# KrishnaswamyLab/MELD

Measured on AMD Instinct MI355X. Metric: cells/sec through MELD.fit_transform (kNN+Chebyshev), higher is better.
Workload: dtype f64

## Files before the change

include/meld_hip.h:

```cpp
#ifndef MELD_HIP_H
#define MELD_HIP_H

#include <stddef.h>
#include <stdint.h>

#ifdef __cplusplus
extern "C" {
#endif

#define MELD_OK 0
#define MELD_ERR_INVALID (-1)
#define MELD_ERR_UNSUPPORTED (-2)
#define MELD_ERR_HIP (-3)

typedef void* meld_stream_t;

int meld_abi_version(void);
const char* meld_last_error(void);
int meld_device_count(void);


int meld_knn_padded_dim(int d);
int meld_knn_tile_refs(void);
int meld_knn_block_queries(void);
// ... 82 lines not shown
                                 const void* Rt16, const float* thr_seed, const float* q_norm2, int nprod, void* temp, void* scratch,
                                 uint32_t* list, int64_t list_stride, int32_t* cnt, int lead_only, meld_stream_t stream);
int meld_knn16_step_lists_direct_spheres(const double* X, int64_t N, int d, const double* mean, const float* scale_info, const float* norm2_max,
                                 const void* Rt16, const float* thr_seed, const float* q_norm2, int nprod, void* temp, void* scratch,
                                 uint32_t* list, int64_t list_stride, int32_t* cnt, int lead_only, meld_stream_t stream);
int meld_knn16_topk_listed(const void* Q16, const float* Qn, const void* Rt16, const float* scale_info, int64_t n_ref, int d,
                           int64_t q_count, int ksel, const uint32_t* step_list, const int32_t* step_cnt, int64_t list_stride,
                           const float* norm2_max, int64_t q_begin, const float* thr_init, int knn, double radius_factor,
                           int32_t* cand_idx, float* cand_d2, int32_t* cand_cnt, float* cand_thr, uint64_t* tiles_done,
                           const int32_t* block_order, int n_slices , meld_stream_t stream);
int meld_knn16_topk_listed_partial(const void* Q16, const float* Qn, const void* Rt16, const float* scale_info, int64_t n_ref,
                                   int d, int64_t q_count, int ksel, const uint32_t* step_list, const int32_t* step_cnt,
                                   int64_t list_stride, const float* norm2_max, int64_t q_begin, const float* thr_init, int knn,
                                   double radius_factor, int32_t* cand_idx, float* cand_d2, int32_t* cand_cnt, float* cand_thr,
                                   uint64_t* tiles_done, const int32_t* block_order, int n_slices, int partial_test,
                                   meld_stream_t stream);
int meld_knn16_partial_filter(const void* Q16, const float* Qn, const void* Rt16, const float* scale_info, const float* norm2_max, int d,
                              int64_t q_count, const float* thr_init, uint32_t* step_list, const int32_t* step_cnt, int64_t list_stride,
                              int32_t* cnt_out, uint64_t* tested, const int32_t* block_order , meld_stream_t stream);
int meld_knn16_resident_blocks(int d, int nprod);
int meld_knn16_max_slices(int ksel);
int meld_knn16_merge_slices(const int32_t* s_idx, const float* s_d2, const int32_t* s_cnt, int64_t q_count,
                            int ksel, int n_slices, int32_t* out_idx, float* out_d2, int32_t* out_cnt,
                            meld_stream_t stream);


int meld_knn_refine(const double* X, int64_t N, int d, int64_t q_begin, int64_t q_count,
                    const int32_t* cand_idx, const float* cand_d2, const int32_t* cand_cnt,
                    const float* cand_thr ,
                    int ksel, int cap , int knn, double decay, double thresh,
                    const float* norm2_max, double err_coef,
                    const float* norm2 , double err_coef_lin, double* bw,
                    double* cand_val, int32_t* keep_cnt, int32_t* flag_rows, int32_t* n_flag,
                    const int32_t* rows, int out_cap, int32_t* cand_idx_out,
// ... 190 lines not shown
```

meld_amd/_lib.py:

```python
from __future__ import annotations

from ._options import is_set, opt

import ctypes as C
import os

_HERE = os.path.dirname(os.path.abspath(__file__))
LIB_NAME = "libmeld_hip.so"
LIB_PATH = os.path.join(_HERE, LIB_NAME)

_i32, _i64, _f64, _sz, _ptr = C.c_int, C.c_int64, C.c_double, C.c_size_t, C.c_void_p

SIGNATURES = {
    "meld_abi_version": (_i32, []),
    "meld_last_error": (C.c_char_p, []),
    "meld_device_count": (_i32, []),
    "meld_knn_padded_dim": (_i32, [_i32]),
    "meld_knn_tile_refs": (_i32, []),
    "meld_knn_block_queries": (_i32, []),
    "meld_knn_row_capacity": (_i32, [_i32]),
    "meld_col_sums_f64": (_i32, [_ptr, _i64, _i32, _ptr, _ptr]),
    "meld_col_stats_temp_bytes": (_sz, [_i32]),
    "meld_col_stats_f64": (_i32, [_ptr, _i64, _i32, _ptr, _ptr, _ptr, _ptr, _sz, _ptr]),
    "meld_knn_prepare_refs": (_i32, [_ptr, _i64, _i32, _ptr, _i32, _ptr, _ptr, _ptr, _ptr]),
# ... 24 lines not shown
    "meld_knn16_bounds_bytes": (_sz, [_i64, _i64]),
    "meld_knn16_bounds_temp_bytes": (_sz, [_i64, _i32, _i64]),
    "meld_knn16_bounds": (_i32, [_ptr, _i64, _i32, _ptr, _ptr, _ptr, _ptr, _i64, _i64, _ptr, _ptr, _i32, _ptr, _ptr, _ptr]),
    "meld_knn16_bounds_from_spheres": (_i32, [_ptr, _i64, _i32, _ptr, _ptr, _ptr, _ptr, _i64, _i64, _ptr, _ptr, _i32, _ptr, _ptr, _ptr]),
    "meld_knn16_tile_spheres": (_i32, [_ptr, _i64, _i32, _ptr, _ptr, _ptr, _i64, _i64, _ptr]),
    "meld_knn16_sphere_layout": (_i32, [_i64, _i32, _ptr, _ptr]),
    "meld_knn16_topk": (_i32, [_ptr, _ptr, _ptr, _ptr, _i64, _i32, _i64, _i32, _i32, _i32, _ptr, _ptr, _i64, _ptr, _i32, _f64, _ptr, _ptr, _ptr, _ptr, _ptr, _ptr, _ptr]),
    "meld_knn16_block_work": (_i32, [_ptr, _ptr, _i64, _i32, _i64, _i32, _ptr, _ptr, _ptr, _ptr]),
    "meld_knn16_step_lists": (_i32, [_ptr, _ptr, _i64, _i32, _i64, _i32, _ptr, _ptr, _i64, _ptr, _i64, _ptr, _ptr]),
    "meld_knn16_list_scratch_bytes": (_sz, [_i64]),
    "meld_knn16_step_lists_direct": (_i32, [_ptr, _i64, _i32, _ptr, _ptr, _ptr, _ptr, _ptr, _ptr, _i32, _ptr, _ptr, _ptr, _i64, _ptr, _ptr]),
    "meld_knn16_prepare_fused": (_i32, [_ptr, _i64, _i32, _ptr, _ptr, _ptr, _ptr, _ptr, _ptr, _ptr, _ptr, _ptr, _ptr, _ptr]),
    "meld_knn16_step_lists_direct_spheres": (_i32, [_ptr, _i64, _i32, _ptr, _ptr, _ptr, _ptr, _ptr, _ptr, _i32, _ptr, _ptr, _ptr, _i64, _ptr, _i32, _ptr]),
    "meld_knn16_step_lists_direct_lead": (_i32, [_ptr, _i64, _i32, _ptr, _ptr, _ptr, _ptr, _ptr, _ptr, _i32, _ptr, _ptr, _ptr, _i64, _ptr, _i32, _ptr]),
    "meld_knn16_topk_listed": (_i32, [_ptr, _ptr, _ptr, _ptr, _i64, _i32, _i64, _i32, _ptr, _ptr, _i64, _ptr, _i64, _ptr, _i32, _f64, _ptr, _ptr, _ptr, _ptr, _ptr, _ptr, _i32, _ptr]),
    "meld_knn16_topk_listed_partial": (_i32, [_ptr, _ptr, _ptr, _ptr, _i64, _i32, _i64, _i32, _ptr, _ptr, _i64, _ptr, _i64, _ptr, _i32, _f64, _ptr, _ptr, _ptr, _ptr, _ptr, _ptr, _i32, _i32, _ptr]),
    "meld_knn16_partial_filter": (_i32, [_ptr, _ptr, _ptr, _ptr, _ptr, _i32, _i64, _ptr, _ptr, _ptr, _i64, _ptr, _ptr, _ptr, _ptr]),
    "meld_knn16_seed_thresholds_mfma": (_i32, [_ptr, _ptr, _ptr, _ptr, _ptr, _i64, _i32, _i64, _i64, _i32, _f64, _i32, _i32, _ptr, _ptr]),
    "meld_knn16_max_slices": (_i32, [_i32]),
    "meld_knn16_merge_slices": (_i32, [_ptr, _ptr, _ptr, _i64, _i32, _i32, _ptr, _ptr, _ptr, _ptr]),
    "meld_knn_radius_exact": (
        _i32,
        [_ptr, _i64, _i32, _i64, _ptr, _i32, _ptr, _i32, _f64, _f64, _i32, _ptr, _ptr, _ptr, _ptr, _ptr, _ptr, _f64, _ptr],
    ),
    "meld_knn_pair_distances": (_i32, [_ptr, _i32, _ptr, _ptr, _i64, _i32, _ptr, _ptr]),
    "meld_metric_tile_rows": (_i32, []),
    "meld_metric_tile_boxes": (_i32, [_ptr, _i64, _i32, _ptr, _ptr, _ptr]),
    "meld_metric_topk": (_i32, [_ptr, _i64, _i32, _i32, _i32, _ptr, _ptr, _i32, _ptr, _ptr, _ptr, _ptr, _ptr, _ptr, _ptr]),
    "meld_metric_refine": (_i32, [_ptr, _ptr, _ptr, _i64, _i32, _i32, _f64, _f64, _ptr, _ptr, _ptr, _ptr, _ptr, _ptr]),
    "meld_metric_radius": (_i32, [_ptr, _i64, _i32, _i32, _ptr, _i32, _ptr, _f64, _f64, _i32, _ptr, _ptr, _ptr, _ptr, _ptr, _ptr]),
    "meld_scan_temp_bytes": (_sz, [_i64]),
    "meld_exclusive_scan_i32_i64": (_i32, [_ptr, _ptr, _i64, _ptr, _sz, _ptr]),
# ... 123 lines not shown
```

meld_amd/csrc/knn16.hip:

```cpp
#include "common.hpp"

#include <hip/hip_fp16.h>

#include <algorithm>

namespace meld {

constexpr int K16_TS = 64;
constexpr int K16_BQ = 256;
constexpr int K16_THREADS = 256;
constexpr int K16_NWAVE = K16_THREADS / 64;
constexpr int K16_SLACK = 128;
constexpr int K16_CAPMAX = 256;
constexpr int K16_BOUNDS_THREADS = 1024;
constexpr int K16_SLOTS = K16_CAPMAX / 64;
constexpr int K16_DMAX = 16 * 9 - 3;

constexpr int K16_SPLIT_DA = 13;
__host__ __device__ inline void k16_slot(int c, int d, int dA, int* coord, int* piece) {
  *coord = -1;
  *piece = -1;
  if (dA == 0) {
    if (c < d) *coord = c;
    else if (c < d + 3) *piece = 3 + (c - d);
// ... 186 lines not shown
  const float* thr_init;
  int knn1;
  float rf2, err_c, err_l;
  int* cand_idx;
  float* cand_d2;
  int* cand_cnt;
  float* cand_thr;
  unsigned long long* tiles_done;
  const int* block_order;
  const unsigned* step_list;
  const int* step_cnt;
  long long list_stride;
  int ee_hi;
  int planes_used;
  int count_go;
};
#define K16_COLD(FIELD) \
  (((const volatile K16Args __attribute__((address_space(4)))*)__builtin_amdgcn_kernarg_segment_ptr())->FIELD)

__host__ __device__ constexpr int k16_waves(int KB, int NPROD, bool EE) {
  return ((NPROD == 1 && KB <= 4) ? 3 : ((KB <= 5 || (NPROD == 1 && KB <= 8)) ? 2 : 1)) + ((EE && KB <= 4) ? 1 : 0);
}

template <int KB, int STATS, int NPROD, bool LIST = false, bool EE = false>
__global__ __launch_bounds__(K16_THREADS)
__attribute__((amdgpu_waves_per_eu(k16_waves(KB, NPROD, EE), k16_waves(KB, NPROD, EE)))) void knn16_topk_kernel(const K16Args a) {
  const _Float16* __restrict__ Q16 = a.Q16;
  const float* __restrict__ Qn = a.Qn;
  const _Float16* __restrict__ Rt16 = a.Rt16;
  const int n_tiles = a.n_tiles, ksel = a.ksel, cap = a.cap;
// ... 21 lines not shown
  const int tid = threadIdx.x;
  const int lane = tid & 63;
  const int wave = __builtin_amdgcn_readfirstlane(tid >> 6);
  const int jq = lane & 31;
  const int h = lane >> 5;
  const int bx = a.block_order ? __builtin_amdgcn_readfirstlane(a.block_order[blockIdx.y]) : (int)blockIdx.y;
  const int q_base = bx * K16_BQ + wave * 64;
  int sl_n_ = (int)gridDim.x;
  asm volatile("" : "+s"(sl_n_));
  const int sl_n = sl_n_, sl_y = (int)blockIdx.x;
  typedef const __attribute__((address_space(4))) unsigned* k16_list_ptr;
  const k16_list_ptr my_list = LIST ? (k16_list_ptr)(uintptr_t)(a.step_list + (size_t)bx * (size_t)a.list_stride) : (k16_list_ptr)0;
  const int n_scan = ((LIST ? __builtin_amdgcn_readfirstlane(a.step_cnt[bx]) : n_tiles) - sl_y + sl_n - 1) / sl_n;
  auto list_entry = [&](int s_) __attribute__((always_inline)) { return s_ < n_scan ? my_list[sl_y + sl_n * s_] : 0u; };
  auto entry_live = [&](unsigned e) __attribute__((always_inline)) { return ((e >> (24 + wave)) & 1u) != 0u; };
  const int row_base = (int)(blockIdx.x * (gridDim.y * K16_BQ)) + q_base;
  float* const wave_d2 = cand_d2 + (size_t)row_base * cap;
  int* const wave_idx = cand_idx + (size_t)row_base * cap;

  f16x8 bhi[2][KB], blo[2][KB];
#pragma unroll
  for (int g = 0; g < 2; ++g) {
    const f16x8* qrow = reinterpret_cast<const f16x8*>(Q16 + (size_t)(q_base + g * 32 + jq) * (KB * 32));
#pragma unroll
    for (int kb = 0; kb < KB; ++kb) {
      bhi[g][kb] = qrow[(kb * 2 + h) * 2 + 0];
      if (NPROD == 3) blo[g][kb] = qrow[(kb * 2 + h) * 2 + 1];
    }
  }
  const float* const wave_qn = Qn + q_base;
// ... 304 lines not shown
        __syncthreads();
      }
      K16_COLD_REGION_END();
    }
    if (any == 0) {
      *live = false;
      return n_scan;
    }
    const int i = (int)__ffsll((long long)any) - 1;
    *live = (my_live >> i) & 1ull;
    win_rem &= ~((2ull << i) - 1ull);
    return win_base + i;
  };

  int n_done = 0;
  auto ee_tile = [&](const _Float16* tile_r, int t) __attribute__((always_inline)) {
    const f16x8* a8 = reinterpret_cast<const f16x8*>(tile_r) + jq;
    const f16x8 aA = a8[h * K16_TS], aB = a8[32 + h * K16_TS];
    const float tA0 = thrp[0] + ee_c[0], tA1 = thrp[1] + ee_c[1];
#pragma unroll
    for (int sub = 0; sub < 2; ++sub) {
#pragma unroll
      for (int r = 0; r < 16; ++r) accA0[r] = accA1[r] = 0.0f;
      accA0 = __builtin_amdgcn_mfma_f32_32x32x16_f16(sub ? aB : aA, bhi[0][0], accA0, 0, 0, 0);
      accA1 = __builtin_amdgcn_mfma_f32_32x32x16_f16(sub ? aB : aA, bhi[1][0], accA1, 0, 0, 0);
      if (__any(min16(accA0) < tA0 || min16(accA1) < tA1)) {
        const f16x8* as = a8 + sub * 32;
#pragma unroll
        for (int kb = 1; kb < KB; ++kb) {
          const f16x8 ahi = as[(kb * 2 + h) * K16_TS];
          accA0 = __builtin_amdgcn_mfma_f32_32x32x16_f16(ahi, bhi[0][kb], accA0, 0, 0, 0);
          accA1 = __builtin_amdgcn_mfma_f32_32x32x16_f16(ahi, bhi[1][kb], accA1, 0, 0, 0);
        }
        const float m0 = min16(accA0), m1 = min16(accA1);
        if (__any(m0 < thrp[0] || m1 < thrp[1])) {
          const unsigned t0s = tm_now();
          select(accA0, accA1, m0, m1, t * K16_TS + 32 * sub + 4 * h);
          if (STATS) {
            const unsigned dsel = tm_now() - t0s;
            tm_sel += dsel;
            tm_mark += dsel;
          }
        }
        ++st_go;
      }
    }
    ++n_done;
  };
  int s_cur = 0;
// ... 20 lines not shown
      K16_LOAD(__builtin_amdgcn_readfirstlane(t_next), (unsigned)TILE_LDS_BYTES);
      K16_STAGED_BUT_LAST();
    } else {
      K16_STAGED();
    }
    K16_TILE_BARRIER();
  }
  unsigned rd_b = 0u, nx_b = (unsigned)TILE_LDS_BYTES, wr_b = 2u * (unsigned)TILE_LDS_BYTES;
  auto scan_step = [&]() __attribute__((always_inline)) {
    const int t = t_cur;
    const _Float16* tile_r = reinterpret_cast<const _Float16*>(reinterpret_cast<const char*>(lds_ring) + rd_b);
    const bool tm_live = live_cur;
    unsigned e_far = 0u;
    if constexpr (LIST) e_far = list_entry(s_next + 2);
    if (EE && live_cur) {
      ee_tile(tile_r, t);
    } else if (live_cur) {
      segment(tile_r, 0, accA0, accA1, accB0, accB1, refB, true, pend);
      segment(tile_r, 1, accB0, accB1, accA0, accA1, t * K16_TS + 4 * h, true, true);
      refB = t * K16_TS + 32 + 4 * h;
      pend = true;
      ++n_done;
    } else if (pend) {
      segment(nullptr, 0, accA0, accA1, accB0, accB1, refB, false, true);
      pend = false;
    }

    if (tm_live) tm_lap(tm_seg); else tm_lap(tm_idle);
    if (batch_every > 0 && (it & (batch_every - 1)) == batch_every - 1) {
      const int limit = ksel + K16_COLD(batch_slack);
      unsigned long long todo = 0;
// ... 48 lines not shown
    live_cur = live_next;
    s_next = s_nn;
    t_next = t_nn;
    live_next = live_nn;
    par ^= 1;
    ++it;
    const unsigned free_b = rd_b;
    rd_b = nx_b;
    nx_b = wr_b;
    wr_b = free_b;
  };
  tm_mark = tm_now();
  if constexpr (PAIR) {
    constexpr unsigned PB = 2u * (unsigned)TILE_LDS_BYTES;
    const int n_pairs = (n_scan + 1) >> 1;
    unsigned c0 = list_entry(0), c1 = list_entry(1), x0 = list_entry(2), x1 = list_entry(3);
    if (n_scan > 0) K16_LOAD(__builtin_amdgcn_readfirstlane((int)(c0 & 0xFFFFFFu)), 0u);
    if (n_scan > 1) K16_LOAD(__builtin_amdgcn_readfirstlane((int)(c1 & 0xFFFFFFu)), (unsigned)TILE_LDS_BYTES);
    K16_STAGED();
    K16_TILE_BARRIER();
    for (int p = 0; p < n_pairs; ++p) {
      const unsigned buf = (p & 1) ? PB : 0u, other = PB - buf;
      const unsigned f0 = list_entry(2 * p + 4), f1 = list_entry(2 * p + 5);
      if (2 * p + 2 < n_scan) K16_LOAD(__builtin_amdgcn_readfirstlane((int)(x0 & 0xFFFFFFu)), other);
      if (2 * p + 3 < n_scan) K16_LOAD(__builtin_amdgcn_readfirstlane((int)(x1 & 0xFFFFFFu)), other + (unsigned)TILE_LDS_BYTES);
      tm_lap(tm_tail);
      const char* ring = reinterpret_cast<const char*>(lds_ring);
      const bool live0 = entry_live(c0), live1 = 2 * p + 1 < n_scan && entry_live(c1);
      if (live0) ee_tile(reinterpret_cast<const _Float16*>(ring + buf), (int)(c0 & 0xFFFFFFu));
      if (live1) ee_tile(reinterpret_cast<const _Float16*>(ring + buf + TILE_LDS_BYTES), (int)(c1 & 0xFFFFFFu));
      if (live0 || live1) tm_lap(tm_seg); else tm_lap(tm_idle);
      if (batch_every > 0 && (p & (batch_every / 2 - 1)) == batch_every / 2 - 1) {
        const int limit = ksel + K16_COLD(batch_slack);
        unsigned long long todo = 0;
#pragma unroll
        for (int g = 0; g < 2; ++g) {
          const int cg = g ? cnt[1] : cnt[0];
          const int tot = cg + __shfl_xor(cg, 32, 64);
          todo |= (__ballot(tot > limit) & 0xffffffffull) << (32 * g);
        }
        while (todo) {
          const int j = __ffsll((long long)todo) - 1;
          todo &= todo - 1;
          squeeze(j >> 5, j & 31);
          if (STATS) ++st_sq;
        }
      }
      tm_lap(tm_tail);
      K16_STAGED();
      tm_lap(tm_dma);
      K16_TILE_BARRIER();
      tm_lap(tm_bar);
      c0 = x0;
      c1 = x1;
      x0 = f0;
      x1 = f1;
      ++it;
    }
  }
  while (!PAIR && s_cur < n_scan) scan_step();
  if (pend) segment(nullptr, 0, accA0, accA1, accB0, accB1, refB, false, true);
  {
    unsigned long long* tiles_done = K16_COLD(tiles_done);
    if (tiles_done && lane == 0) {
      atomicAdd(tiles_done, (unsigned long long)n_done);
      if (EE && K16_COLD(count_go)) atomicAdd(tiles_done + 1, (unsigned long long)st_go);
    }
  }

  unsigned long long* stats = STATS ? K16_COLD(stats) : nullptr;
  if (STATS && stats) {
// ... 32 lines not shown
    }
  }
#undef K16_LOAD
#undef K16_DMA
#undef K16_STAGED
#undef K16_STAGED_BUT_LAST
#undef K16_TILE_BARRIER
#undef K16_ROUND_OK
}

template <int TPS, int WPE>
__global__ __launch_bounds__(256) __attribute__((amdgpu_waves_per_eu(WPE, WPE))) void knn16_partial_filter_kernel(const _Float16* __restrict__ Q16, const float* __restrict__ Qn,
                                                                   const _Float16* __restrict__ Rt16, const float* __restrict__ scale_info,
                                                                   const float* __restrict__ norm2_max, const float* __restrict__ thr_init,
                                                                   unsigned* step_list, const int* __restrict__ step_cnt, long long list_stride,
                                                                   int* __restrict__ cnt_out, unsigned long long* __restrict__ tested,
                                                                   const int* __restrict__ block_order, int KB, int ee_hi) {
  static_assert(TPS >= 2 && TPS <= 32 && (TPS & 1) == 0, "tiles per step");
  __shared__ __attribute__((aligned(16))) _Float16 ring[2][TPS][2 * K16_TS * 8];
  __shared__ unsigned wmask[2][4];
  const int tid = threadIdx.x, lane = tid & 63;
  const int wave = __builtin_amdgcn_readfirstlane(tid >> 6);
  const int jq = lane & 31, h = lane >> 5;
  const int bx = block_order ? __builtin_amdgcn_readfirstlane(block_order[blockIdx.x]) : (int)blockIdx.x;
  const int q_base = bx * K16_BQ + wave * 64;
  f16x8 b0[2];
  float tA[2];
  {
    const float s_ = scale_info[0];
    const float delta = 3.814697265625e-06f * (norm2_max[0] * s_ * s_) + 1e-30f;
#pragma unroll
    for (int g = 0; g < 2; ++g) {
      const int q = q_base + g * 32 + jq;
      const f16x8* qrow = reinterpret_cast<const f16x8*>(Q16 + (size_t)q * (size_t)(KB * 32));
      b0[g] = qrow[h * 2];
      float qb = 0.0f;
      for (int kb = 1; kb < KB; ++kb) {
        const f16x8 v8 = qrow[(kb * 2 + h) * 2];
#pragma unroll
        for (int e = 0; e < 8; ++e) {
          const float v = (16 * kb + 8 * h + e < ee_hi) ? (float)v8[e] : 0.0f;
          qb = fmaf(v, v, qb);
        }
      }
      qb += __shfl_xor(qb, 32, 64);
      tA[g] = (thr_init[q] - Qn[q]) + (qb * 1.0001f + delta);
    }
  }
  unsigned* const my_list_w = step_list + (size_t)bx * (size_t)list_stride;
  const int n = __builtin_amdgcn_readfirstlane(step_cnt[bx]);
  const int n_steps = (n + TPS - 1) / TPS;
  const size_t tile_bytes = (size_t)KB * 4096;
  const int plane_stride = 2048;
  const size_t src_base = reinterpret_cast<size_t>(Rt16);
  typedef __attribute__((address_space(3))) void* lds_ptr_t;
  typedef int i32x4 __attribute__((ext_vector_type(4)));
  const unsigned ring_base = (unsigned)(size_t)(lds_ptr_t)&ring[0][0][0];
  const int lane16 = lane * 16;
  auto load_entries = [&](int step) __attribute__((always_inline)) {
    const int idx = step * TPS + lane;
    return (lane < TPS && idx < n) ? my_list_w[idx] : 0u;
  };
  auto stage = [&](unsigned ev, int buf) __attribute__((always_inline)) {
#pragma unroll
// ... 1 lines not shown
      const int k = wave * (TPS / 2) + u;
      const unsigned e = (unsigned)__builtin_amdgcn_readlane((int)ev, k >> 1);
      if (e >> 24) {
        const size_t src = src_base + (size_t)(e & 0xFFFFFFu) * tile_bytes;
        const i32x4 rsrc = {(int)(unsigned)src, (int)((src >> 32) & 0xffffu), 4096, 0x00020000};
        asm volatile("s_mov_b32 m0, %0\n\ts_nop 0\n\tbuffer_load_dwordx4 %1, %2, %3 offen lds" ::"s"(__builtin_amdgcn_readfirstlane(
                         (int)(ring_base + (unsigned)((buf * TPS + (k >> 1)) * 2048 + (k & 1) * 1024)))),
                     "v"(lane16), "s"(rsrc), "s"((k & 1) * plane_stride)
                     : "memory");
      }
    }
  };
  int out_n = 0;
  unsigned long long n_tested = 0;
  auto emit = [&](unsigned ev, int par) __attribute__((always_inline)) {
    unsigned nm = 0u;
#pragma unroll
    for (int w = 0; w < 4; ++w) nm |= ((wmask[par][w] >> lane) & 1u) << w;
    nm &= (ev >> 24);
    const bool keep = nm != 0u;
    const unsigned long long b = __ballot(keep);
    if (keep) my_list_w[out_n + __popcll(b & ((1ull << lane) - 1ull))] = (ev & 0xFFFFFFu) | (nm << 24);
    out_n += __popcll(b);
  };
  unsigned ev_prev = 0u, ev_cur = load_entries(0), ev_nxt = load_entries(1);
  if (n_steps > 0) stage(ev_cur, 0);
  __builtin_amdgcn_s_waitcnt(0x0F70);
  asm volatile("s_waitcnt lgkmcnt(0)\n\ts_barrier" ::: "memory");
  for (int s = 0; s < n_steps; ++s) {
    const int buf = s & 1;
    const unsigned ev_nn = load_entries(s + 2);
    if (s + 1 < n_steps) stage(ev_nxt, buf ^ 1);
    if (wave == 0 && s > 0) emit(ev_prev, buf ^ 1);
    unsigned mybits = 0u;
#pragma unroll
    for (int j = 0; j < TPS; ++j) {
      const unsigned e = (unsigned)__builtin_amdgcn_readlane((int)ev_cur, j);
      if ((e >> (24 + wave)) & 1u) {
        const f16x8* a8 = reinterpret_cast<const f16x8*>(&ring[buf][j][0]) + jq;
        const f16x8 aA = a8[h * K16_TS], aB = a8[h * K16_TS + 32];
        f32x16 c00, c01, c10, c11;
#pragma unroll
        for (int r = 0; r < 16; ++r) c00[r] = c01[r] = c10[r] = c11[r] = 0.0f;
        c00 = __builtin_amdgcn_mfma_f32_32x32x16_f16(aA, b0[0], c00, 0, 0, 0);
        c01 = __builtin_amdgcn_mfma_f32_32x32x16_f16(aA, b0[1], c01, 0, 0, 0);
        c10 = __builtin_amdgcn_mfma_f32_32x32x16_f16(aB, b0[0], c10, 0, 0, 0);
        c11 = __builtin_amdgcn_mfma_f32_32x32x16_f16(aB, b0[1], c11, 0, 0, 0);
        const bool hit = __builtin_fminf(min16(c00), min16(c10)) < tA[0] || __builtin_fminf(min16(c01), min16(c11)) < tA[1];
        if (__any(hit)) mybits |= 1u << j;
        ++n_tested;
      }
    }
    if (lane == 0) wmask[buf][wave] = mybits;
    __builtin_amdgcn_s_waitcnt(0x0F70);
    asm volatile("s_waitcnt lgkmcnt(0)\n\ts_barrier" ::: "memory");
    ev_prev = ev_cur;
    ev_cur = ev_nxt;
    ev_nxt = ev_nn;
  }
  if (wave == 0) {
    if (n_steps > 0) emit(ev_prev, (n_steps - 1) & 1);
    if (lane == 0) cnt_out[bx] = out_n;
  }
  if (tested && lane == 0) atomicAdd(tested, n_tested);
}

template <int SL>
__device__ __forceinline__ void k16_bitonic_sort(unsigned long long (&key)[SL], int lane) {
// ... 1421 lines not shown
    }
    hipLaunchKernelGGL((knn16_topk_kernel<KB, STATS, 1, true>), grid, dim3(K16_THREADS), 0, st, ka);
  } else if (nprod == 1) {
    hipLaunchKernelGGL((knn16_topk_kernel<KB, STATS, 1>), grid, dim3(K16_THREADS), 0, st, ka);
  } else {
    hipLaunchKernelGGL((knn16_topk_kernel<KB, STATS, 3>), grid, dim3(K16_THREADS), 0, st, ka);
  }
}

static int k16_topk_impl(const void* Q16, const float* Qn, const void* Rt16, const float* scale_info,
                         int64_t n_ref, int d,
                         int64_t q_count, int ksel, int nprod, int n_slices, const void* lb2,
                         const float* norm2_max, int64_t q_begin, const float* thr_init, int knn,
                         double radius_factor, int32_t* cand_idx, float* cand_d2, int32_t* cand_cnt,
                         float* cand_thr, uint64_t* tiles_done, const int32_t* block_order, const uint32_t* step_list,
                         const int32_t* step_cnt, int64_t list_stride, meld_stream_t stream, int partial_test = 0, int two_counters = 0) {
  MELD_CHECK_ARG(nprod == 1 || nprod == 3, "meld_knn16_topk: nprod must be 1 or 3");
  MELD_CHECK_ARG(step_list == nullptr || (step_cnt != nullptr && nprod == 1 && lb2 == nullptr && thr_init != nullptr),
                 "meld_knn16_topk_listed: step lists go with the hi-only pass, start thresholds and no table");
  MELD_CHECK_ARG(n_slices >= 1 && n_slices * ksel <= K16_MERGE_MAX, "meld_knn16_topk: n_slices=%d must satisfy n_slices * ksel <= %d",
                 n_slices, K16_MERGE_MAX);
  MELD_CHECK_ARG(Q16 && Qn && Rt16 && scale_info && cand_idx && cand_d2 && cand_cnt, "meld_knn16_topk: null pointer");
  MELD_CHECK_ARG(lb2 == nullptr || norm2_max != nullptr, "meld_knn16_topk: pruning needs norm2_max");
  MELD_CHECK_ARG(cand_thr == nullptr || (norm2_max != nullptr && knn >= 0 && knn < ksel && radius_factor >= 1.0),
                 "meld_knn16_topk: the radius cut needs norm2_max, 0 <= knn < ksel, radius_factor >= 1");
  const int knn1 = (cand_thr && knn >= 1) ? knn + 1 : 0;
  const float rf2 = knn1 > 0 ? (float)(radius_factor * radius_factor * (1.0 + 1e-6)) : 0.0f;
  const float err_c = (float)meld_knn16_error_coef_const(nprod, d), err_l = (float)meld_knn16_error_coef_lin(nprod);
  MELD_CHECK_ARG(n_ref > 0 && n_ref < (int64_t)1 << 31 && q_count > 0, "meld_knn16_topk: bad sizes");
  const int cap = meld_knn16_row_capacity(ksel);
  if (cap < 0) return cap;
// ... 39 lines not shown
  ka.err_c = err_c;
  ka.err_l = err_l;
  ka.cand_idx = cand_idx;
  ka.cand_d2 = cand_d2;
  ka.cand_cnt = cand_cnt;
  ka.cand_thr = cand_thr;
  ka.tiles_done = reinterpret_cast<unsigned long long*>(tiles_done);
  ka.block_order = block_order;
  ka.step_list = step_list;
  ka.step_cnt = step_cnt;
  ka.list_stride = (long long)list_stride;
  const int dA = k16_dA(d, KB);
  const bool ee = step_list != nullptr && dA > 0 && KB >= 2 && KB <= 7 && partial_test != 0;
  ka.ee_hi = 16 + d - dA;
  ka.count_go = two_counters;
  ka.planes_used = ((dA > 0 ? 16 + (d - dA) + 3 : d + 3) + 7) / 8;
#define K16_CASE(KBV)                                                                                                      \
  case KBV:                                                                                                                \
    (stats ? k16_launch_topk<KBV, 1> : k16_launch_topk<KBV, 0>)(grid, S(stream), ka, step_list != nullptr, ee, nprod); \
    break;
  switch (KB) {
    K16_CASE(1)
    K16_CASE(2)
    K16_CASE(3)
    K16_CASE(4)
    K16_CASE(5)
    K16_CASE(6)
    K16_CASE(7)
    K16_CASE(8)
    K16_CASE(9)
// ... 42 lines not shown
                                      int d, int64_t q_count, int ksel, const uint32_t* step_list, const int32_t* step_cnt,
                                      int64_t list_stride, const float* norm2_max, int64_t q_begin, const float* thr_init, int knn,
                                      double radius_factor, int32_t* cand_idx, float* cand_d2, int32_t* cand_cnt, float* cand_thr,
                                      uint64_t* tiles_done, const int32_t* block_order, int n_slices, meld_stream_t stream) {
  MELD_CHECK_ARG(step_list && step_cnt && list_stride > 0, "meld_knn16_topk_listed: null step lists");
  return k16_topk_impl(Q16, Qn, Rt16, scale_info, n_ref, d, q_count, ksel, 1, n_slices, nullptr, norm2_max, q_begin, thr_init, knn,
                       radius_factor, cand_idx, cand_d2, cand_cnt, cand_thr, tiles_done, block_order, step_list, step_cnt, list_stride,
                       stream);
}

extern "C" int meld_knn16_topk_listed_partial(const void* Q16, const float* Qn, const void* Rt16, const float* scale_info, int64_t n_ref,
                                              int d, int64_t q_count, int ksel, const uint32_t* step_list, const int32_t* step_cnt,
                                              int64_t list_stride, const float* norm2_max, int64_t q_begin, const float* thr_init, int knn,
                                              double radius_factor, int32_t* cand_idx, float* cand_d2, int32_t* cand_cnt, float* cand_thr,
                                              uint64_t* tiles_done, const int32_t* block_order, int n_slices, int partial_test,
                                              meld_stream_t stream) {
  MELD_CHECK_ARG(step_list && step_cnt && list_stride > 0, "meld_knn16_topk_listed_partial: null step lists");
  return k16_topk_impl(Q16, Qn, Rt16, scale_info, n_ref, d, q_count, ksel, 1, n_slices, nullptr, norm2_max, q_begin, thr_init, knn,
                       radius_factor, cand_idx, cand_d2, cand_cnt, cand_thr, tiles_done, block_order, step_list, step_cnt, list_stride,
                       stream, partial_test, 1);
}

extern "C" int meld_knn16_partial_filter(const void* Q16, const float* Qn, const void* Rt16, const float* scale_info, const float* norm2_max,
                                         int d, int64_t q_count, const float* thr_init, uint32_t* step_list, const int32_t* step_cnt,
                                         int64_t list_stride, int32_t* cnt_out, uint64_t* tested, const int32_t* block_order,
                                         meld_stream_t stream) {
  MELD_CHECK_ARG(Q16 && Qn && Rt16 && scale_info && norm2_max && thr_init && step_list && step_cnt && cnt_out && list_stride > 0 && q_count > 0,
                 "meld_knn16_partial_filter: null pointer or bad sizes");
  const int KB = meld_knn16_kblocks(d);
  if (KB < 0) return KB;
  const int dA = k16_dA(d, KB);
  MELD_CHECK_ARG(dA > 0 && KB >= 2, "meld_knn16_partial_filter: d = %d has no split operand layout", d);
  const unsigned n_blocks = (unsigned)ceil_div(q_count, K16_BQ);
  hipLaunchKernelGGL((knn16_partial_filter_kernel<8, 4>), dim3(n_blocks), dim3(256), 0, S(stream), reinterpret_cast<const _Float16*>(Q16), Qn,
                     reinterpret_cast<const _Float16*>(Rt16), scale_info, norm2_max, thr_init, step_list, step_cnt, (long long)list_stride, cnt_out,
                     reinterpret_cast<unsigned long long*>(tested), block_order, KB, 16 + d - dA);
  MELD_LAUNCH_CHECK("knn16_partial_filter_kernel");
  return MELD_OK;
}

extern "C" int meld_knn16_resident_blocks(int d, int nprod) {
  MELD_CHECK_ARG(nprod == 1 || nprod == 3, "meld_knn16_resident_blocks: nprod must be 1 or 3");
  const int KB = meld_knn16_kblocks(d);
  if (KB < 0) return KB;
  int per_cu = 0;
#define K16_OCC(KBV)                                                                                              \
  case KBV:                                                                                                       \
    if (nprod == 1) {                                                                                             \
      MELD_HIP_CALL(hipOccupancyMaxActiveBlocksPerMultiprocessor(&per_cu, knn16_topk_kernel<KBV, 0, 1>, K16_THREADS, 0)); \
    } else {                                                                                                      \
      MELD_HIP_CALL(hipOccupancyMaxActiveBlocksPerMultiprocessor(&per_cu, knn16_topk_kernel<KBV, 0, 3>, K16_THREADS, 0)); \
// ... 38 lines not shown
```

meld_amd/graph.py:

```python
from __future__ import annotations

from ._options import opt

import math
import time

from types import SimpleNamespace

import numpy as np
import torch

from ._lib import check, get_lib, ptr
from .knn_plan import SearchOptions, plan_knn_search, search_nprod, sphere_layout

__all__ = ["DeviceGraph", "build_knn_graph", "default_ksel", "EVENTS", "record_events"]

EVENTS = {"enabled": False, "pairs": []}


def record_events(enabled=True):
    EVENTS["enabled"] = bool(enabled)
    EVENTS["pairs"] = []


# ... 655 lines not shown
                check(lib.meld_knn16_step_lists(ptr(lb2), ptr(seeds), N, d, a.q_count, plan.nprod, ptr(nmax), ptr(o.scale_info), a.q_begin,
                                                ptr(step_list), n_tiles, ptr(step_cnt), st), "meld_knn16_step_lists")
        work = step_cnt
        if plan.block_order == "work":
            work = torch.empty(n_blocks, dtype=torch.int32, device=dev)
            check(lib.meld_knn16_block_work(ptr(lb2), ptr(seeds), N, d, a.q_count, plan.nprod, ptr(nmax), ptr(o.scale_info), ptr(work), st), "meld_knn16_block_work")
        block_order = torch.argsort(work, descending=True, stable=True).to(torch.int32) if plan.block_order != "none" else None
        a.tm.stop("bounds")
        return lb2, step_list, step_cnt, block_order

    def _search16(self, a, plan, o, c, ksel, seeds, rfac, lists):
        lib, st, dev, d, q_count, q_pad, cap = self.lib, _stream(), a.X.device, a.d, a.q_count, o.q_pad, c.cap
        lb2, step_list, step_cnt, block_order = lists
        q0 = 0 if a.cross else a.q_begin
        tiles_b = c.tiles_done
        if plan.two_pass:
            with _EventSpan("knn_filter", N=a.N, d=d, q=q_count):
                check(lib.meld_knn16_partial_filter(ptr(o.Q), ptr(o.Qn), ptr(o.Rt), ptr(o.scale_info), ptr(c.nmax), d, q_count, ptr(seeds), ptr(step_list),
                                                    ptr(step_cnt), o.n_tiles, ptr(step_cnt), ptr(c.tiles_done), ptr(block_order), st), "meld_knn16_partial_filter")
                if block_order is not None:
                    block_order = torch.argsort(step_cnt, descending=True, stable=True).to(torch.int32)
            tiles_b = c.tiles_done[1:]
            a.tm.stop("knn_filter")
        S = plan.main_slices
        with _EventSpan("knn_topk", N=a.N, d=d, q=q_count):
            if S > 1:
                out = (torch.empty(S * q_pad * cap, dtype=torch.int32, device=dev), torch.empty(S * q_pad * cap, dtype=torch.float32, device=dev),
                       torch.empty(S * q_pad, dtype=torch.int32, device=dev), torch.full((S, q_pad), float("inf"), dtype=torch.float32, device=dev))
            else:
                out = (c.idx, c.d2, c.cnt, c.thr)
            if step_list is not None:
                check(lib.meld_knn16_topk_listed_partial(ptr(o.Q), ptr(o.Qn), ptr(o.Rt), ptr(o.scale_info), a.NR, d, q_count, ksel, ptr(step_list), ptr(step_cnt),
                                                         o.n_tiles, ptr(c.nmax), q0, ptr(seeds), plan.knn_cut, rfac, *map(ptr, out), ptr(tiles_b), ptr(block_order),
                                                         S, int(plan.partial_in_search), st), "meld_knn16_topk_listed")
            else:
                check(lib.meld_knn16_topk(ptr(o.Q), ptr(o.Qn), ptr(o.Rt), ptr(o.scale_info), a.NR, d, q_count, ksel, plan.nprod, S, ptr(lb2), ptr(c.nmax), q0,
                                          ptr(seeds), plan.knn_cut, rfac, *map(ptr, out), ptr(c.tiles_done), ptr(block_order), st), "meld_knn16_topk")
            if S > 1:
                check(lib.meld_knn16_merge_slices(*map(ptr, out[:3]), q_count, ksel, S, ptr(c.idx), ptr(c.d2), ptr(c.cnt), st), "meld_knn16_merge_slices")
                c.thr.copy_(out[3].amin(0))
            del out
            while _WHILE_SEARCHING:
                _WHILE_SEARCHING.pop()()
        del o.Q

    def _refine(self, a, c, ksel):
        lib, st, dev, q_count = self.lib, _stream(), a.X.device, a.q_count
        r = SimpleNamespace(plan=c.plan, cands=c)
        max_rank = 0 if a.knn_max is None else int(a.knn_max) + 1
# ... 671 lines not shown
```

Before: 28.67 million.

## Record per-quadrant filter hits and skip dead sub-tile MFMAs in search

The partial filter kernel now records a 4-bit mask per tile showing which 32x32 quadrants (query half by reference half) passed the threshold test, and stores it in a new step_sub array alongside the step list. The early-exit search kernel reads these nibbles and only loads A fragments and runs MFMA chains for live quadrants, skipping whole sub-blocks or one of the two accumulators. This cuts tensor-core work and LDS reads in the main top-k pass. In exchange it adds an extra buffer allocation, a 16-bit write per listed tile, extra loads and branching in the pipelined loop, and more divergence in the kernel's control flow.

```diff
diff --git a/include/meld_hip.h b/include/meld_hip.h
--- a/include/meld_hip.h
+++ b/include/meld_hip.h
@@ -120,10 +120,12 @@
                                    int64_t list_stride, const float* norm2_max, int64_t q_begin, const float* thr_init, int knn,
                                    double radius_factor, int32_t* cand_idx, float* cand_d2, int32_t* cand_cnt, float* cand_thr,
                                    uint64_t* tiles_done, const int32_t* block_order, int n_slices, int partial_test,
+                                   const uint16_t* step_sub ,
                                    meld_stream_t stream);
 int meld_knn16_partial_filter(const void* Q16, const float* Qn, const void* Rt16, const float* scale_info, const float* norm2_max, int d,
                               int64_t q_count, const float* thr_init, uint32_t* step_list, const int32_t* step_cnt, int64_t list_stride,
-                              int32_t* cnt_out, uint64_t* tested, const int32_t* block_order , meld_stream_t stream);
+                              int32_t* cnt_out, uint16_t* step_sub , uint64_t* tested,
+                              const int32_t* block_order , meld_stream_t stream);
 int meld_knn16_resident_blocks(int d, int nprod);
 int meld_knn16_max_slices(int ksel);
 int meld_knn16_merge_slices(const int32_t* s_idx, const float* s_d2, const int32_t* s_cnt, int64_t q_count,
diff --git a/meld_amd/_lib.py b/meld_amd/_lib.py
--- a/meld_amd/_lib.py
+++ b/meld_amd/_lib.py
@@ -62,8 +62,8 @@
     "meld_knn16_step_lists_direct_spheres": (_i32, [_ptr, _i64, _i32, _ptr, _ptr, _ptr, _ptr, _ptr, _ptr, _i32, _ptr, _ptr, _ptr, _i64, _ptr, _i32, _ptr]),
     "meld_knn16_step_lists_direct_lead": (_i32, [_ptr, _i64, _i32, _ptr, _ptr, _ptr, _ptr, _ptr, _ptr, _i32, _ptr, _ptr, _ptr, _i64, _ptr, _i32, _ptr]),
     "meld_knn16_topk_listed": (_i32, [_ptr, _ptr, _ptr, _ptr, _i64, _i32, _i64, _i32, _ptr, _ptr, _i64, _ptr, _i64, _ptr, _i32, _f64, _ptr, _ptr, _ptr, _ptr, _ptr, _ptr, _i32, _ptr]),
-    "meld_knn16_topk_listed_partial": (_i32, [_ptr, _ptr, _ptr, _ptr, _i64, _i32, _i64, _i32, _ptr, _ptr, _i64, _ptr, _i64, _ptr, _i32, _f64, _ptr, _ptr, _ptr, _ptr, _ptr, _ptr, _i32, _i32, _ptr]),
-    "meld_knn16_partial_filter": (_i32, [_ptr, _ptr, _ptr, _ptr, _ptr, _i32, _i64, _ptr, _ptr, _ptr, _i64, _ptr, _ptr, _ptr, _ptr]),
+    "meld_knn16_topk_listed_partial": (_i32, [_ptr, _ptr, _ptr, _ptr, _i64, _i32, _i64, _i32, _ptr, _ptr, _i64, _ptr, _i64, _ptr, _i32, _f64, _ptr, _ptr, _ptr, _ptr, _ptr, _ptr, _i32, _i32, _ptr, _ptr]),
+    "meld_knn16_partial_filter": (_i32, [_ptr, _ptr, _ptr, _ptr, _ptr, _i32, _i64, _ptr, _ptr, _ptr, _i64, _ptr, _ptr, _ptr, _ptr, _ptr]),
     "meld_knn16_seed_thresholds_mfma": (_i32, [_ptr, _ptr, _ptr, _ptr, _ptr, _i64, _i32, _i64, _i64, _i32, _f64, _i32, _i32, _ptr, _ptr]),
     "meld_knn16_max_slices": (_i32, [_i32]),
     "meld_knn16_merge_slices": (_i32, [_ptr, _ptr, _ptr, _i64, _i32, _i32, _ptr, _ptr, _ptr, _ptr]),
diff --git a/meld_amd/csrc/knn16.hip b/meld_amd/csrc/knn16.hip
--- a/meld_amd/csrc/knn16.hip
+++ b/meld_amd/csrc/knn16.hip
@@ -224,6 +224,7 @@
   int ee_hi;
   int planes_used;
   int count_go;
+  const unsigned short* step_sub;
 };
 #define K16_COLD(FIELD) \
   (((const volatile K16Args __attribute__((address_space(4)))*)__builtin_amdgcn_kernarg_segment_ptr())->FIELD)
@@ -275,6 +276,15 @@
   const int n_scan = ((LIST ? __builtin_amdgcn_readfirstlane(a.step_cnt[bx]) : n_tiles) - sl_y + sl_n - 1) / sl_n;
   auto list_entry = [&](int s_) __attribute__((always_inline)) { return s_ < n_scan ? my_list[sl_y + sl_n * s_] : 0u; };
   auto entry_live = [&](unsigned e) __attribute__((always_inline)) { return ((e >> (24 + wave)) & 1u) != 0u; };
+  const uintptr_t my_sub = (LIST && EE && a.step_sub) ? (uintptr_t)(a.step_sub + (size_t)bx * (size_t)a.list_stride) : (uintptr_t)0;
+  auto sub_addr = [&](int s_) __attribute__((always_inline)) { return my_sub + 2u * (uintptr_t)(unsigned)(sl_y + sl_n * s_); };
+  auto sub_word = [&](int s_) __attribute__((always_inline)) {
+    return (my_sub != 0 && s_ < n_scan) ? *(k16_list_ptr)(sub_addr(s_) & ~(uintptr_t)3) : 0xFFFFFFFFu;
+  };
+  auto sub_entry = [&](unsigned e, unsigned w, int s_) __attribute__((always_inline)) {
+    const unsigned nib = (w >> (8u * ((unsigned)sub_addr(s_) & 2u) + 4u * (unsigned)wave)) & 15u;
+    return (e & 0xFFFFFFu) | (entry_live(e) ? nib << 24 : 0u);
+  };
   const int row_base = (int)(blockIdx.x * (gridDim.y * K16_BQ)) + q_base;
   float* const wave_d2 = cand_d2 + (size_t)row_base * cap;
   int* const wave_idx = cand_idx + (size_t)row_base * cap;
@@ -609,25 +619,55 @@
   };
 
   int n_done = 0;
-  auto ee_tile = [&](const _Float16* tile_r, int t) __attribute__((always_inline)) {
+  auto ee_tile = [&](const _Float16* tile_r, int t, unsigned quad) __attribute__((always_inline)) {
     const f16x8* a8 = reinterpret_cast<const f16x8*>(tile_r) + jq;
-    const f16x8 aA = a8[h * K16_TS], aB = a8[32 + h * K16_TS];
+    f16x8 aA = __builtin_nondeterministic_value(aA), aB = __builtin_nondeterministic_value(aB);
+    if (quad & 3u) aA = a8[h * K16_TS];
+    if (quad & 12u) aB = a8[32 + h * K16_TS];
     const float tA0 = thrp[0] + ee_c[0], tA1 = thrp[1] + ee_c[1];
 #pragma unroll
     for (int sub = 0; sub < 2; ++sub) {
-#pragma unroll
-      for (int r = 0; r < 16; ++r) accA0[r] = accA1[r] = 0.0f;
-      accA0 = __builtin_amdgcn_mfma_f32_32x32x16_f16(sub ? aB : aA, bhi[0][0], accA0, 0, 0, 0);
-      accA1 = __builtin_amdgcn_mfma_f32_32x32x16_f16(sub ? aB : aA, bhi[1][0], accA1, 0, 0, 0);
-      if (__any(min16(accA0) < tA0 || min16(accA1) < tA1)) {
-        const f16x8* as = a8 + sub * 32;
-#pragma unroll
-        for (int kb = 1; kb < KB; ++kb) {
-          const f16x8 ahi = as[(kb * 2 + h) * K16_TS];
-          accA0 = __builtin_amdgcn_mfma_f32_32x32x16_f16(ahi, bhi[0][kb], accA0, 0, 0, 0);
-          accA1 = __builtin_amdgcn_mfma_f32_32x32x16_f16(ahi, bhi[1][kb], accA1, 0, 0, 0);
+      const unsigned lv = (quad >> (2 * sub)) & 3u;
+      if (lv == 0u) continue;
+      const f16x8* as = a8 + sub * 32;
+      bool go;
+      if (lv == 3u) {
+#pragma unroll
+        for (int r = 0; r < 16; ++r) accA0[r] = accA1[r] = 0.0f;
+        accA0 = __builtin_amdgcn_mfma_f32_32x32x16_f16(sub ? aB : aA, bhi[0][0], accA0, 0, 0, 0);
+        accA1 = __builtin_amdgcn_mfma_f32_32x32x16_f16(sub ? aB : aA, bhi[1][0], accA1, 0, 0, 0);
+        go = __any(min16(accA0) < tA0 || min16(accA1) < tA1);
+        if (go) {
+#pragma unroll
+          for (int kb = 1; kb < KB; ++kb) {
+            const f16x8 ahi = as[(kb * 2 + h) * K16_TS];
+            accA0 = __builtin_amdgcn_mfma_f32_32x32x16_f16(ahi, bhi[0][kb], accA0, 0, 0, 0);
+            accA1 = __builtin_amdgcn_mfma_f32_32x32x16_f16(ahi, bhi[1][kb], accA1, 0, 0, 0);
+          }
         }
-        const float m0 = min16(accA0), m1 = min16(accA1);
+      } else if (lv == 1u) {
+        accA1 = __builtin_nondeterministic_value(accA1);
+#pragma unroll
+        for (int r = 0; r < 16; ++r) accA0[r] = 0.0f;
+        accA0 = __builtin_amdgcn_mfma_f32_32x32x16_f16(sub ? aB : aA, bhi[0][0], accA0, 0, 0, 0);
+        go = __any(min16(accA0) < tA0);
+        if (go) {
+#pragma unroll
+          for (int kb = 1; kb < KB; ++kb) accA0 = __builtin_amdgcn_mfma_f32_32x32x16_f16(as[(kb * 2 + h) * K16_TS], bhi[0][kb], accA0, 0, 0, 0);
+        }
+      } else {
+        accA0 = __builtin_nondeterministic_value(accA0);
+#pragma unroll
+        for (int r = 0; r < 16; ++r) accA1[r] = 0.0f;
+        accA1 = __builtin_amdgcn_mfma_f32_32x32x16_f16(sub ? aB : aA, bhi[1][0], accA1, 0, 0, 0);
+        go = __any(min16(accA1) < tA1);
+        if (go) {
+#pragma unroll
+          for (int kb = 1; kb < KB; ++kb) accA1 = __builtin_amdgcn_mfma_f32_32x32x16_f16(as[(kb * 2 + h) * K16_TS], bhi[1][kb], accA1, 0, 0, 0);
+        }
+      }
+      if (go) {
+        const float m0 = (lv & 1u) ? min16(accA0) : INFINITY, m1 = (lv & 2u) ? min16(accA1) : INFINITY;
         if (__any(m0 < thrp[0] || m1 < thrp[1])) {
           const unsigned t0s = tm_now();
           select(accA0, accA1, m0, m1, t * K16_TS + 32 * sub + 4 * h);
@@ -678,7 +718,7 @@
     unsigned e_far = 0u;
     if constexpr (LIST) e_far = list_entry(s_next + 2);
     if (EE && live_cur) {
-      ee_tile(tile_r, t);
+      ee_tile(tile_r, t, 15u);
     } else if (live_cur) {
       segment(tile_r, 0, accA0, accA1, accB0, accB1, refB, true, pend);
       segment(tile_r, 1, accB0, accB1, accA0, accA1, t * K16_TS + 4 * h, true, true);
@@ -757,7 +797,8 @@
   if constexpr (PAIR) {
     constexpr unsigned PB = 2u * (unsigned)TILE_LDS_BYTES;
     const int n_pairs = (n_scan + 1) >> 1;
-    unsigned c0 = list_entry(0), c1 = list_entry(1), x0 = list_entry(2), x1 = list_entry(3);
+    unsigned c0 = sub_entry(list_entry(0), sub_word(0), 0), c1 = sub_entry(list_entry(1), sub_word(1), 1);
+    unsigned x0 = sub_entry(list_entry(2), sub_word(2), 2), x1 = sub_entry(list_entry(3), sub_word(3), 3);
     if (n_scan > 0) K16_LOAD(__builtin_amdgcn_readfirstlane((int)(c0 & 0xFFFFFFu)), 0u);
     if (n_scan > 1) K16_LOAD(__builtin_amdgcn_readfirstlane((int)(c1 & 0xFFFFFFu)), (unsigned)TILE_LDS_BYTES);
     K16_STAGED();
@@ -765,13 +806,14 @@
     for (int p = 0; p < n_pairs; ++p) {
       const unsigned buf = (p & 1) ? PB : 0u, other = PB - buf;
       const unsigned f0 = list_entry(2 * p + 4), f1 = list_entry(2 * p + 5);
+      unsigned fw0 = sub_word(2 * p + 4), fw1 = sub_word(2 * p + 5);
       if (2 * p + 2 < n_scan) K16_LOAD(__builtin_amdgcn_readfirstlane((int)(x0 & 0xFFFFFFu)), other);
       if (2 * p + 3 < n_scan) K16_LOAD(__builtin_amdgcn_readfirstlane((int)(x1 & 0xFFFFFFu)), other + (unsigned)TILE_LDS_BYTES);
       tm_lap(tm_tail);
       const char* ring = reinterpret_cast<const char*>(lds_ring);
-      const bool live0 = entry_live(c0), live1 = 2 * p + 1 < n_scan && entry_live(c1);
-      if (live0) ee_tile(reinterpret_cast<const _Float16*>(ring + buf), (int)(c0 & 0xFFFFFFu));
-      if (live1) ee_tile(reinterpret_cast<const _Float16*>(ring + buf + TILE_LDS_BYTES), (int)(c1 & 0xFFFFFFu));
+      const bool live0 = (c0 >> 24) != 0u, live1 = 2 * p + 1 < n_scan && (c1 >> 24) != 0u;
+      if (live0) ee_tile(reinterpret_cast<const _Float16*>(ring + buf), (int)(c0 & 0xFFFFFFu), c0 >> 24);
+      if (live1) ee_tile(reinterpret_cast<const _Float16*>(ring + buf + TILE_LDS_BYTES), (int)(c1 & 0xFFFFFFu), c1 >> 24);
       if (live0 || live1) tm_lap(tm_seg); else tm_lap(tm_idle);
       if (batch_every > 0 && (p & (batch_every / 2 - 1)) == batch_every / 2 - 1) {
         const int limit = ksel + K16_COLD(batch_slack);
@@ -796,8 +838,9 @@
       tm_lap(tm_bar);
       c0 = x0;
       c1 = x1;
-      x0 = f0;
-      x1 = f1;
+      asm volatile("" : "+s"(fw0), "+s"(fw1));
+      x0 = sub_entry(f0, fw0, 2 * p + 4);
+      x1 = sub_entry(f1, fw1, 2 * p + 5);
       ++it;
     }
   }
@@ -860,11 +903,13 @@
                                                                    const _Float16* __restrict__ Rt16, const float* __restrict__ scale_info,
                                                                    const float* __restrict__ norm2_max, const float* __restrict__ thr_init,
                                                                    unsigned* step_list, const int* __restrict__ step_cnt, long long list_stride,
-                                                                   int* __restrict__ cnt_out, unsigned long long* __restrict__ tested,
+                                                                   int* __restrict__ cnt_out, unsigned short* __restrict__ step_sub,
+                                                                   unsigned long long* __restrict__ tested,
                                                                    const int* __restrict__ block_order, int KB, int ee_hi) {
   static_assert(TPS >= 2 && TPS <= 32 && (TPS & 1) == 0, "tiles per step");
   __shared__ __attribute__((aligned(16))) _Float16 ring[2][TPS][2 * K16_TS * 8];
-  __shared__ unsigned wmask[2][4];
+  constexpr int WM = (TPS + 7) / 8;
+  __shared__ unsigned wmask[2][4][WM];
   const int tid = threadIdx.x, lane = tid & 63;
   const int wave = __builtin_amdgcn_readfirstlane(tid >> 6);
   const int jq = lane & 31, h = lane >> 5;
@@ -894,6 +939,7 @@
     }
   }
   unsigned* const my_list_w = step_list + (size_t)bx * (size_t)list_stride;
+  unsigned short* const my_sub_w = step_sub ? step_sub + (size_t)bx * (size_t)list_stride : nullptr;
   const int n = __builtin_amdgcn_readfirstlane(step_cnt[bx]);
   const int n_steps = (n + TPS - 1) / TPS;
   const size_t tile_bytes = (size_t)KB * 4096;
@@ -925,13 +971,22 @@
   int out_n = 0;
   unsigned long long n_tested = 0;
   auto emit = [&](unsigned ev, int par) __attribute__((always_inline)) {
-    unsigned nm = 0u;
-#pragma unroll
-    for (int w = 0; w < 4; ++w) nm |= ((wmask[par][w] >> lane) & 1u) << w;
+    unsigned nm = 0u, sq = 0u;
+    const int jl = lane < TPS ? lane : 0;
+#pragma unroll
+    for (int w = 0; w < 4; ++w) {
+      const unsigned nib = (wmask[par][w][jl >> 3] >> (4 * (jl & 7))) & 15u;
+      nm |= (nib != 0u ? 1u : 0u) << w;
+      sq |= nib << (4 * w);
+    }
     nm &= (ev >> 24);
     const bool keep = nm != 0u;
     const unsigned long long b = __ballot(keep);
-    if (keep) my_list_w[out_n + __popcll(b & ((1ull << lane) - 1ull))] = (ev & 0xFFFFFFu) | (nm << 24);
+    if (keep) {
+      const int pos = out_n + __popcll(b & ((1ull << lane) - 1ull));
+      my_list_w[pos] = (ev & 0xFFFFFFu) | (nm << 24);
+      if (my_sub_w) my_sub_w[pos] = (unsigned short)sq;
+    }
     out_n += __popcll(b);
   };
   unsigned ev_prev = 0u, ev_cur = load_entries(0), ev_nxt = load_entries(1);
@@ -943,7 +998,9 @@
     const unsigned ev_nn = load_entries(s + 2);
     if (s + 1 < n_steps) stage(ev_nxt, buf ^ 1);
     if (wave == 0 && s > 0) emit(ev_prev, buf ^ 1);
-    unsigned mybits = 0u;
+    unsigned mybits[WM];
+#pragma unroll
+    for (int k = 0; k < WM; ++k) mybits[k] = 0u;
 #pragma unroll
     for (int j = 0; j < TPS; ++j) {
       const unsigned e = (unsigned)__builtin_amdgcn_readlane((int)ev_cur, j);
@@ -957,12 +1014,16 @@
         c01 = __builtin_amdgcn_mfma_f32_32x32x16_f16(aA, b0[1], c01, 0, 0, 0);
         c10 = __builtin_amdgcn_mfma_f32_32x32x16_f16(aB, b0[0], c10, 0, 0, 0);
         c11 = __builtin_amdgcn_mfma_f32_32x32x16_f16(aB, b0[1], c11, 0, 0, 0);
-        const bool hit = __builtin_fminf(min16(c00), min16(c10)) < tA[0] || __builtin_fminf(min16(c01), min16(c11)) < tA[1];
-        if (__any(hit)) mybits |= 1u << j;
+        const unsigned q = (__any(min16(c00) < tA[0]) ? 1u : 0u) | (__any(min16(c01) < tA[1]) ? 2u : 0u) | (__any(min16(c10) < tA[0]) ? 4u : 0u) |
+                           (__any(min16(c11) < tA[1]) ? 8u : 0u);
+        mybits[j >> 3] |= q << (4 * (j & 7));
         ++n_tested;
       }
     }
-    if (lane == 0) wmask[buf][wave] = mybits;
+    if (lane == 0) {
+#pragma unroll
+      for (int k = 0; k < WM; ++k) wmask[buf][wave][k] = mybits[k];
+    }
     __builtin_amdgcn_s_waitcnt(0x0F70);
     asm volatile("s_waitcnt lgkmcnt(0)\n\ts_barrier" ::: "memory");
     ev_prev = ev_cur;
@@ -2414,7 +2475,8 @@
                          const float* norm2_max, int64_t q_begin, const float* thr_init, int knn,
                          double radius_factor, int32_t* cand_idx, float* cand_d2, int32_t* cand_cnt,
                          float* cand_thr, uint64_t* tiles_done, const int32_t* block_order, const uint32_t* step_list,
-                         const int32_t* step_cnt, int64_t list_stride, meld_stream_t stream, int partial_test = 0, int two_counters = 0) {
+                         const int32_t* step_cnt, int64_t list_stride, meld_stream_t stream, int partial_test = 0, int two_counters = 0,
+                         const uint16_t* step_sub = nullptr) {
   MELD_CHECK_ARG(nprod == 1 || nprod == 3, "meld_knn16_topk: nprod must be 1 or 3");
   MELD_CHECK_ARG(step_list == nullptr || (step_cnt != nullptr && nprod == 1 && lb2 == nullptr && thr_init != nullptr),
                  "meld_knn16_topk_listed: step lists go with the hi-only pass, start thresholds and no table");
@@ -2484,6 +2546,8 @@
   const bool ee = step_list != nullptr && dA > 0 && KB >= 2 && KB <= 7 && partial_test != 0;
   ka.ee_hi = 16 + d - dA;
   ka.count_go = two_counters;
+  MELD_CHECK_ARG(step_sub == nullptr || (reinterpret_cast<uintptr_t>(step_sub) & 3u) == 0, "meld_knn16_topk_listed_partial: step_sub must be 4-byte aligned");
+  ka.step_sub = ee ? step_sub : nullptr;
   ka.planes_used = ((dA > 0 ? 16 + (d - dA) + 3 : d + 3) + 7) / 8;
 #define K16_CASE(KBV)                                                                                                      \
   case KBV:                                                                                                                \
@@ -2556,17 +2620,17 @@
                                               int64_t list_stride, const float* norm2_max, int64_t q_begin, const float* thr_init, int knn,
                                               double radius_factor, int32_t* cand_idx, float* cand_d2, int32_t* cand_cnt, float* cand_thr,
                                               uint64_t* tiles_done, const int32_t* block_order, int n_slices, int partial_test,
-                                              meld_stream_t stream) {
+                                              const uint16_t* step_sub, meld_stream_t stream) {
   MELD_CHECK_ARG(step_list && step_cnt && list_stride > 0, "meld_knn16_topk_listed_partial: null step lists");
   return k16_topk_impl(Q16, Qn, Rt16, scale_info, n_ref, d, q_count, ksel, 1, n_slices, nullptr, norm2_max, q_begin, thr_init, knn,
                        radius_factor, cand_idx, cand_d2, cand_cnt, cand_thr, tiles_done, block_order, step_list, step_cnt, list_stride,
-                       stream, partial_test, 1);
+                       stream, partial_test, 1, step_sub);
 }
 
 extern "C" int meld_knn16_partial_filter(const void* Q16, const float* Qn, const void* Rt16, const float* scale_info, const float* norm2_max,
                                          int d, int64_t q_count, const float* thr_init, uint32_t* step_list, const int32_t* step_cnt,
-                                         int64_t list_stride, int32_t* cnt_out, uint64_t* tested, const int32_t* block_order,
-                                         meld_stream_t stream) {
+                                         int64_t list_stride, int32_t* cnt_out, uint16_t* step_sub, uint64_t* tested,
+                                         const int32_t* block_order, meld_stream_t stream) {
   MELD_CHECK_ARG(Q16 && Qn && Rt16 && scale_info && norm2_max && thr_init && step_list && step_cnt && cnt_out && list_stride > 0 && q_count > 0,
                  "meld_knn16_partial_filter: null pointer or bad sizes");
   const int KB = meld_knn16_kblocks(d);
@@ -2576,7 +2640,7 @@
   const unsigned n_blocks = (unsigned)ceil_div(q_count, K16_BQ);
   hipLaunchKernelGGL((knn16_partial_filter_kernel<8, 4>), dim3(n_blocks), dim3(256), 0, S(stream), reinterpret_cast<const _Float16*>(Q16), Qn,
                      reinterpret_cast<const _Float16*>(Rt16), scale_info, norm2_max, thr_init, step_list, step_cnt, (long long)list_stride, cnt_out,
-                     reinterpret_cast<unsigned long long*>(tested), block_order, KB, 16 + d - dA);
+                     step_sub, reinterpret_cast<unsigned long long*>(tested), block_order, KB, 16 + d - dA);
   MELD_LAUNCH_CHECK("knn16_partial_filter_kernel");
   return MELD_OK;
 }
diff --git a/meld_amd/graph.py b/meld_amd/graph.py
--- a/meld_amd/graph.py
+++ b/meld_amd/graph.py
@@ -693,10 +693,13 @@
         lb2, step_list, step_cnt, block_order = lists
         q0 = 0 if a.cross else a.q_begin
         tiles_b = c.tiles_done
+        step_sub = None
         if plan.two_pass:
+            step_sub = torch.empty((step_list.numel() + 1) & ~1, dtype=torch.int16, device=dev)
             with _EventSpan("knn_filter", N=a.N, d=d, q=q_count):
                 check(lib.meld_knn16_partial_filter(ptr(o.Q), ptr(o.Qn), ptr(o.Rt), ptr(o.scale_info), ptr(c.nmax), d, q_count, ptr(seeds), ptr(step_list),
-                                                    ptr(step_cnt), o.n_tiles, ptr(step_cnt), ptr(c.tiles_done), ptr(block_order), st), "meld_knn16_partial_filter")
+                                                    ptr(step_cnt), o.n_tiles, ptr(step_cnt), ptr(step_sub), ptr(c.tiles_done), ptr(block_order), st),
+                      "meld_knn16_partial_filter")
                 if block_order is not None:
                     block_order = torch.argsort(step_cnt, descending=True, stable=True).to(torch.int32)
             tiles_b = c.tiles_done[1:]
@@ -711,7 +714,7 @@
             if step_list is not None:
                 check(lib.meld_knn16_topk_listed_partial(ptr(o.Q), ptr(o.Qn), ptr(o.Rt), ptr(o.scale_info), a.NR, d, q_count, ksel, ptr(step_list), ptr(step_cnt),
                                                          o.n_tiles, ptr(c.nmax), q0, ptr(seeds), plan.knn_cut, rfac, *map(ptr, out), ptr(tiles_b), ptr(block_order),
-                                                         S, int(plan.partial_in_search), st), "meld_knn16_topk_listed")
+                                                         S, int(plan.partial_in_search), ptr(step_sub), st), "meld_knn16_topk_listed")
             else:
                 check(lib.meld_knn16_topk(ptr(o.Q), ptr(o.Qn), ptr(o.Rt), ptr(o.scale_info), a.NR, d, q_count, ksel, plan.nprod, S, ptr(lb2), ptr(c.nmax), q0,
                                           ptr(seeds), plan.knn_cut, rfac, *map(ptr, out), ptr(c.tiles_done), ptr(block_order), st), "meld_knn16_topk")
```

Result: slower. 28.09 million (-2.0%).
